# sigma0-dev/polymath

Hardware: AMD Instinct MI355X
Metric: prove_constraints_per_sec (higher is better)
Workload: dtype u32; 1 GPU; 2^20-100-constraint synthetic R1CS (random A*B=C gates), bls12_381, n=2^21, transcript=merlin; msm_pairs_per_proof=29359963, parallelism=one GPU

## Files before the change

polymath_amd/csrc/api.hip:

```cpp
#include <algorithm>
#include <atomic>
#include <cstdlib>
#include <cstring>
#include <exception>
#include <memory>
#include <new>
#include <thread>

#include "internal.h"
#include "comm.h"
#include "fq28.cuh"
#include "../host/hashes.hpp"

using namespace pm;

extern "C" void pm_host_keccak_f1600(uint64_t state[25]) { pmhost::keccak_f1600(state); }

template <class F>
static void parallel_chunks(uint64_t count, F body) {
    unsigned T = std::thread::hardware_concurrency();
    if (T > 32) T = 32;
    if (T < 1 || count < ((uint64_t)1 << 16)) T = 1;
    static const int env_threads = [] { const char *e = getenv("PM_HOST_THREADS"); return e ? std::max(1, atoi(e)) : 0; }();
    if (env_threads) T = (unsigned)env_threads;
// ... 43 lines not shown
struct OptionSpec { const char *env; long long def, lo, hi; };
static const OptionSpec OPTION_SPECS[PM_NUM_OPTIONS] = {
     {"PM_MSM_OVERLAP", 1, 0, 1},
     {"PM_NTT_OVERLAP", 1, 0, 1},
     {"PM_TABLES", PM_TABLES_AUTO, PM_TABLES_OFF, PM_TABLES_NO_WIDE},
     {"PM_MSM_MAX_PIECE_LOG", 27, 4, 27},
     {"PM_MAX_SEG_LOG", 0, 0, 40},
     {"PM_INFLIGHT_CONTEXTS", 1, 1, 64},
     {"PM_MSM_SEG", 0, 0, 1 << 20},
     {"PM_TABLE_C", 0, 0, 24},
     {"PM_WIRE_CHUNK_LOG", 20, 4, 24},
};
static void options_defaults(pm_options *o) {
    for (int k = 0; k < PM_NUM_OPTIONS; ++k) {
        long long v = OPTION_SPECS[k].def;
        if (const char *e = getenv(OPTION_SPECS[k].env)) {
            if (k == PM_OPT_TABLES) v = e[0] == 'w' ? PM_TABLES_WIDE : e[0] == '0' ? PM_TABLES_OFF : PM_TABLES_AUTO;
            else v = atoll(e);
            if (v < OPTION_SPECS[k].lo || v > OPTION_SPECS[k].hi) v = OPTION_SPECS[k].def;
        }
        o->v[k] = v;
    }
    if (o->v[PM_OPT_TABLES] == PM_TABLES_AUTO) {
        const char *e = getenv("PM_WIDE");
        if (e && e[0] == '0') o->v[PM_OPT_TABLES] = PM_TABLES_NO_WIDE;
    }
}

extern "C" int pm_ctx_set_option(pm_ctx *ctx, int option, long long value) {
    if (!ctx || option < 0 || option >= PM_NUM_OPTIONS) return PM_ERR_INVALID_ARG;
    if (value < OPTION_SPECS[option].lo || value > OPTION_SPECS[option].hi) return PM_ERR_INVALID_ARG;
    ctx->opt.v[option] = value;
    if (ctx->aux) ctx->aux->opt.v[option] = value;
    return PM_OK;
}
extern "C" int pm_ctx_get_option(const pm_ctx *ctx, int option, long long *value) {
    if (!ctx || !value || option < 0 || option >= PM_NUM_OPTIONS) return PM_ERR_INVALID_ARG;
    *value = ctx->opt.v[option];
    return PM_OK;
}

extern "C" int pm_ctx_create(int device, pm_ctx **out) {
    if (!out) return PM_ERR_INVALID_ARG;
    *out = nullptr;
    int n = 0;
    if (hipGetDeviceCount(&n) != hipSuccess || n <= 0) return PM_ERR_NO_DEVICE;
    if (device < 0 || device >= n) return PM_ERR_INVALID_ARG;
    pm_ctx *ctx = new (std::nothrow) pm_ctx();
    if (!ctx) return PM_ERR_INVALID_ARG;
    ctx->device = device;
    options_defaults(&ctx->opt);
    ctx->pk = nullptr;
    ctx->phase = 0;
    ctx->aux = nullptr;
    ctx->comm = nullptr;
    ctx->tw_clock = 0;
    ctx->shard_roots_n = 0; ctx->shard_roots_N = 0; ctx->shard_roots_curve = -1;
    ctx->ntt_lds_attr[0] = ctx->ntt_lds_attr[1] = false;
    ctx->h_pinned = nullptr;
    ctx->msm_async = 0;
    ctx->keep_timings = false;
    ctx->lazy_timings = false;
    timing_reset(ctx);
    if (hipSetDevice(device) != hipSuccess || hipStreamCreateWithFlags(&ctx->stream, hipStreamNonBlocking) != hipSuccess) {
        delete ctx;
        return PM_ERR_HIP;
    }
    if (hipEventCreateWithFlags(&ctx->ev_sc_a, hipEventDisableTiming) != hipSuccess) {
        (void)hipStreamDestroy(ctx->stream);
        delete ctx;
        return PM_ERR_HIP;
    }
    *out = ctx;
    return PM_OK;
}

extern "C" void pm_ctx_destroy(pm_ctx *ctx) {
    if (!ctx) return;
    if (ctx->aux) pm_ctx_destroy(ctx->aux);
    (void)hipSetDevice(ctx->device);
    (void)hipStreamSynchronize(ctx->stream);
    timing_flush(ctx);
    MsmWorkspace &m = ctx->msm;
    for (DevBuf *b : {&m.set.sorted, &m.set.counts, &m.set.bucket_off, &m.set.task_off, &m.set.order, &m.set.partials, &m.set.task_cnt}) b->release();
    for (DevBuf *b : {&m.digits, &m.cursor, &m.wsum,
                      &m.region, &m.sub, &m.digits2, &m.len_bins, &m.block_cnt, &m.hot, &ctx->scratch, &ctx->flags, &ctx->xw, &ctx->ue, &ctx->we, &ctx->u, &ctx->w,
                      &ctx->wit_u, &ctx->u2, &ctx->sc_a, &ctx->sc_c, &ctx->quotient, &ctx->ztail, &ctx->ra, &ctx->sh_a, &ctx->sh_b, &ctx->sh_c, &ctx->halo,
                      &ctx->shard_roots, &ctx->ntt_tmp})
        b->release();
    for (auto &b : ctx->lvl) b.release();
    for (auto &b : ctx->fb_table) b.release();
    for (auto &t : ctx->tw) { t.fwd.release(); t.inv.release(); t.fwd_int.release(); t.inv_int.release(); }
    if (ctx->h_pinned) (void)hipHostFree(ctx->h_pinned);
    for (auto &t : ctx->pending_timers) { (void)hipEventDestroy(t.a); (void)hipEventDestroy(t.b); }
    for (hipEvent_t e : ctx->event_pool) (void)hipEventDestroy(e);
    (void)hipEventDestroy(ctx->ev_sc_a);
    (void)hipStreamDestroy(ctx->stream);
    delete ctx;
}

extern "C" const char *pm_last_error(const pm_ctx *ctx) { return ctx ? ctx->err.c_str() : "null context"; }

extern "C" int pm_last_timings(pm_ctx *ctx, double *ms_out, int n_slots) {
    if (!ctx || !ms_out) return PM_ERR_INVALID_ARG;
    if (!ctx->pending_timers.empty()) {
        if (hipSetDevice(ctx->device) != hipSuccess) return PM_ERR_HIP;
        timing_flush_now(ctx);
    }
    for (int i = 0; i < n_slots; ++i) ms_out[i] = i < T_NUM_SLOTS ? ctx->timing_ms[i] : 0.0;
    return PM_OK;
}

template <class C>
static int ntt_host(pm_ctx *ctx, uint64_t *data, unsigned log_n, int inverse) {
    typedef Fp<typename C::FrP> Fr;
    if (log_n > (unsigned)C::TWO_ADICITY) return PM_ERR_DOMAIN_TOO_LARGE;
    size_t bytes = sizeof(Fr) << log_n;
    PM_HIP(ctx, ctx->scratch.reserve(bytes));
    PM_HIP(ctx, hipMemcpyAsync(ctx->scratch.p, data, bytes, hipMemcpyHostToDevice, ctx->stream));
    timing_reset(ctx);
    PM_TRY(ntt_run<C>(ctx, ctx->scratch.as<Fr>(), log_n, inverse != 0));
    PM_HIP(ctx, hipMemcpyAsync(data, ctx->scratch.p, bytes, hipMemcpyDeviceToHost, ctx->stream));
    PM_HIP(ctx, hipStreamSynchronize(ctx->stream));
    timing_flush(ctx);
    return PM_OK;
}

extern "C" int pm_ntt(pm_ctx *ctx, int curve, uint64_t *data, unsigned log_n, int inverse) {
    if (!ctx || !data) return PM_ERR_INVALID_ARG;
    PM_TRY(set_device(ctx));
    return PM_DISPATCH(curve, ntt_host<BlsCurve>(ctx, data, log_n, inverse), ntt_host<BnCurve>(ctx, data, log_n, inverse));
}

template <class C>
static int ntt_dev(pm_ctx *ctx, uint64_t *d, unsigned log_n, int inverse) {
    timing_reset(ctx);
    PM_TRY(ntt_run<C>(ctx, (Fp<typename C::FrP> *)d, log_n, inverse != 0));
    PM_HIP(ctx, hipStreamSynchronize(ctx->stream));
    timing_flush(ctx);
    return PM_OK;
}

extern "C" int pm_ntt_device(pm_ctx *ctx, int curve, uint64_t *d_data, unsigned log_n, int inverse) {
    if (!ctx || !d_data) return PM_ERR_INVALID_ARG;
    PM_TRY(set_device(ctx));
    return PM_DISPATCH(curve, ntt_dev<BlsCurve>(ctx, d_data, log_n, inverse), ntt_dev<BnCurve>(ctx, d_data, log_n, inverse));
}

struct BasesDeleter {
    void operator()(pm_bases *b) const {
        if (!b) return;
        (void)hipSetDevice(b->device);
        if (b->d_points) (void)hipFree(b->d_points);
        if (b->d_inf) (void)hipFree(b->d_inf);
        if (b->d_table) (void)hipFree(b->d_table);
        delete b;
    }
};
typedef std::unique_ptr<pm_bases, BasesDeleter> BasesPtr;

template <class C>
static int bases_upload_impl(pm_ctx *ctx, const void *bases, size_t stride, size_t len, pm_bases **out) {
    if (stride < sizeof(Affine<C>)) return PM_ERR_INVALID_ARG;
    BasesPtr b(new pm_bases{C::ID, ctx->device, len, nullptr});
    if (len) {
        std::vector<Affine<C>> packed(len);
        repack_bases<C>(bases, stride, len, packed.data());
// ... 914 lines not shown
```

polymath_amd/csrc/internal.h:

```cpp
#pragma once
#include <hip/hip_runtime.h>
#include <stdint.h>
#include <stdlib.h>

#include <chrono>
#include <condition_variable>
#include <cstdio>
#include <functional>
#include <mutex>
#include <string>
#include <thread>
#include <vector>

#include "../../include/polymath_hip.h"
#include "../host/layout.hpp"
#include "ec.cuh"

namespace pm {

struct pm_error_sink {
    std::string msg;
};

#define PM_HIP(ctx, expr)                                                                        \
    do {                                                                                         \
        hipError_t _e = (expr);                                                                  \
        if (_e != hipSuccess) {                                                                  \
            (ctx)->err = std::string(#expr) + ": " + hipGetErrorString(_e) + " @" + __FILE__ + ":" + \
                         std::to_string(__LINE__);                                               \
            return PM_ERR_HIP;                                                                   \
        }                                                                                        \
    } while (0)

#define PM_TRY(expr)                  \
    do {                              \
        int _s = (expr);              \
        if (_s != PM_OK) return _s;   \
    } while (0)

struct DevBuf {
    void *p = nullptr;
    size_t bytes = 0;
    hipError_t reserve(size_t need) {
        if (need <= bytes) return hipSuccess;
        if (p) {
            hipError_t e = hipFree(p);
            if (e != hipSuccess) return e;
            p = nullptr;
            bytes = 0;
        }
        size_t want = need + need / 8;
        hipError_t e = hipMalloc(&p, want);
        if (e != hipSuccess) {
            e = hipMalloc(&p, need);
            want = need;
        }
        if (e == hipSuccess) bytes = want;
        return e;
    }
    void release() {
        if (p) (void)hipFree(p);
        p = nullptr;
        bytes = 0;
    }
    template <class T>
    T *as() const { return (T *)p; }
};

enum TimingSlot {
    T_WITNESS_MAP = 0,
    T_NTT = 1,
    T_POLY = 2,
    T_MSM_SORT = 3,
    T_MSM_ACCUMULATE = 4,
    T_MSM_REDUCE = 5,
    T_MSM_TOTAL = 6,
    T_PHASE = 7,
    T_NUM_SLOTS = 8
};

struct MsmSet {
    DevBuf sorted, counts, bucket_off, task_off, order, partials, task_cnt;
};
struct MsmWorkspace {
    MsmSet set;
    DevBuf digits, cursor, wsum, region, sub, digits2, len_bins, block_cnt, hot;
};

struct MsmTables {
    unsigned c = 0, nwin = 0;
    unsigned off[33] = {0};
    unsigned char width[32] = {0};
    size_t stride = 0;
    size_t base_index = 0;
    const unsigned char *inf = nullptr;
    const void *table = nullptr;
    bool wide = false;
};

struct TwiddleCache {
    int curve = -1;
    unsigned log_n = 0;
    unsigned long long stamp = 0;
    DevBuf fwd, inv;
    DevBuf fwd_int, inv_int;
};

}

struct pm_bases {
    int curve;
    int device;
    size_t len;
    void *d_points;
    void *d_inf;
    void *d_table;
    pm::MsmTables tables;
};

struct pm_pk {
    int curve, device;
    uint64_t n, m0, mw, nr, sigma;
    unsigned log_n;
    uint64_t omega[4];
    int shard_rank, shard_count;
    uint64_t *d_rowptr[3];
    uint32_t *d_col[3];
    uint64_t *d_val[3];
    uint64_t nnz[3];
    void *d_bases;
    uint64_t base_len[PM_NUM_BASE_VECS];
    uint64_t seg_off[PM_NUM_BASE_VECS];
    uint64_t total_points;
    uint64_t res_lo[3], res_hi[3], res_dev_off[3];
    uint64_t msm_lo[3], msm_len[3];
    int layout;
    std::vector<pmlayout::Piece> pieces[3];
    uint64_t res_cnt[3];
    std::vector<pmlayout::Segment> segs;
    uint64_t max_seg;
    uint64_t max_piece = (uint64_t)1 << 27;
    struct SegRef { uint64_t a, b; uint32_t rank, idx; };
    std::vector<SegRef> all_segs;
    size_t seg_slots;
    void *d_segs;
    void *d_all_segs = nullptr;
    pm::MsmTables tables[3];
    void *d_tab[3], *d_tab_inf[3];
};

struct pm_worker {
    std::thread th;
    std::mutex mu;
    std::condition_variable cv;
    std::function<void()> job;
    bool has_job = false, done = true, stop = false;
    bool submit(std::function<void()> fn) {
        std::unique_lock<std::mutex> lk(mu);
        if (!th.joinable()) {
            try {
                th = std::thread([this] {
                    std::unique_lock<std::mutex> l(mu);
                    for (;;) {
                        cv.wait(l, [this] { return has_job || stop; });
                        if (stop) return;
// ... 284 lines not shown
```

polymath_amd/csrc/msm.hip:

```cpp
#include <cstdlib>
#include <cstring>

#include "internal.h"
#include "fq28.cuh"

namespace pm {

constexpr uint32_t DIGIT_NONE = 0xFFFFFFFFu;

struct MsmPlan {
    unsigned c, nwin, nbuckets;
    unsigned seg;
    size_t len;
    unsigned chunk, nchunks;
    size_t max_tasks;
};

static MsmPlan make_plan(size_t len, unsigned scalar_bits, unsigned task_len = 0) {
    MsmPlan p;
    p.len = len;
    double best = 1e300;
    unsigned bc = 4;
    for (unsigned c = 4; c <= 16; ++c) {
        unsigned w = (scalar_bits + 1 + c - 1) / c;
// ... 104 lines not shown
        __syncthreads();
        s_a[tid] += va;
        s_b[tid] += vb;
        __syncthreads();
    }
    uint32_t ra = s_a[tid] - sa, rb = s_b[tid] - sb;
#pragma unroll
    for (unsigned k = 0; k < SCAN_PER; ++k) {
        if (base + k < G) { bucket_off[base + k] = ra; task_off[base + k] = rb; }
        ra += c[k];
        rb += nt[k];
    }
    if (tid == 255) { tile_tot[2 * blockIdx.x] = s_a[255]; tile_tot[2 * blockIdx.x + 1] = s_b[255]; }
}

__global__ __launch_bounds__(1024) void k_scan_totals(uint32_t *tile_tot, unsigned ntiles, uint32_t *bucket_off,
                                                      uint32_t *task_off, size_t G) {
    __shared__ uint32_t s_a[1024], s_b[1024];
    const unsigned tid = threadIdx.x;
    uint32_t carry_a = 0, carry_b = 0;
    for (unsigned base = 0; base < ntiles; base += 1024) {
        unsigned i = base + tid;
        uint32_t a = i < ntiles ? tile_tot[2 * i] : 0u, b = i < ntiles ? tile_tot[2 * i + 1] : 0u;
        s_a[tid] = a;
        s_b[tid] = b;
        __syncthreads();
        for (unsigned off = 1; off < 1024; off <<= 1) {
            uint32_t va = 0, vb = 0;
            if (tid >= off) { va = s_a[tid - off]; vb = s_b[tid - off]; }
            __syncthreads();
            s_a[tid] += va;
            s_b[tid] += vb;
            __syncthreads();
        }
        if (i < ntiles) { tile_tot[2 * i] = carry_a + s_a[tid] - a; tile_tot[2 * i + 1] = carry_b + s_b[tid] - b; }
        carry_a += s_a[1023];
        carry_b += s_b[1023];
        __syncthreads();
    }
    if (tid == 0) { bucket_off[G] = carry_a; task_off[G] = carry_b; }
}

__global__ __launch_bounds__(256) void k_scan_add(uint32_t *bucket_off, uint32_t *task_off, const uint32_t *tile_tot, size_t G) {
    const size_t base = (size_t)blockIdx.x * SCAN_TILE + (size_t)threadIdx.x * SCAN_PER;
    const uint32_t oa = tile_tot[2 * blockIdx.x], ob = tile_tot[2 * blockIdx.x + 1];
#pragma unroll
    for (unsigned k = 0; k < SCAN_PER; ++k)
        if (base + k < G) { bucket_off[base + k] += oa; task_off[base + k] += ob; }
}

__global__ __launch_bounds__(1024) void k_scatter(const uint32_t *digits, const uint32_t *bucket_off, uint32_t *cursor,
                                                  uint32_t *sorted, size_t len, unsigned chunk, unsigned nbuckets) {
    extern __shared__ __attribute__((aligned(16))) unsigned char smem_raw[];
    uint32_t *h = (uint32_t *)smem_raw;
    const unsigned w = blockIdx.y;
    for (unsigned b = threadIdx.x; b < nbuckets; b += blockDim.x) h[b] = 0;
    __syncthreads();
    size_t lo = (size_t)blockIdx.x * chunk, hi = lo + chunk;
    if (hi > len) hi = len;
    const uint32_t *d = digits + (size_t)w * len;
    for (size_t i = lo + threadIdx.x; i < hi; i += blockDim.x) {
        uint32_t v = d[i];
        if (v != DIGIT_NONE) atomicAdd(&h[v >> 1], 1u);
    }
    __syncthreads();
    const size_t gbase = (size_t)w * nbuckets;
    for (unsigned b = threadIdx.x; b < nbuckets; b += blockDim.x) {
        uint32_t v = h[b];
        if (v) h[b] = bucket_off[gbase + b] + atomicAdd(&cursor[gbase + b], v);
    }
    __syncthreads();
    for (size_t i = lo + threadIdx.x; i < hi; i += blockDim.x) {
        uint32_t v = d[i];
        if (v != DIGIT_NONE) {
            uint32_t pos = atomicAdd(&h[v >> 1], 1u);
            sorted[pos] = ((uint32_t)i << 1) | (v & 1u);
        }
    }
}

constexpr unsigned TASK_MAX_BINS = 8192;

template <bool SCATTER>
__global__ __launch_bounds__(1024) void k_task_bins(const uint32_t *counts, const uint32_t *task_off, size_t G, unsigned seg,
                                                    unsigned lshift, unsigned nbins, uint32_t *len_cnt, const uint32_t *len_off,
                                                    uint32_t *len_cursor, uint32_t *order) {
    extern __shared__ __attribute__((aligned(16))) unsigned char smem_raw[];
    uint32_t *h = (uint32_t *)smem_raw;
    for (unsigned b = threadIdx.x; b < nbins; b += blockDim.x) h[b] = 0;
    __syncthreads();
    const size_t g = (size_t)blockIdx.x * blockDim.x + threadIdx.x;
    uint32_t t0 = 0, n = 0, rank_full = 0, rank_last = 0;
    unsigned bin = 0;
    if (g < G) {
        t0 = task_off[g];
        n = task_off[g + 1] - t0;
        if (n) {
            const uint32_t L = counts[g] - (n - 1) * seg;
            bin = (seg - L) >> lshift;
            if (n > 1) rank_full = atomicAdd(&h[0], n - 1);
            rank_last = atomicAdd(&h[bin], 1u);
        }
    }
    __syncthreads();
    if (!SCATTER) {
        for (unsigned b = threadIdx.x; b < nbins; b += blockDim.x) {
            const uint32_t v = h[b];
            if (v) atomicAdd(&len_cnt[b], v);
        }
    } else {
        for (unsigned b = threadIdx.x; b < nbins; b += blockDim.x) {
            const uint32_t v = h[b];
            if (v) h[b] = len_off[b] + atomicAdd(&len_cursor[b], v);
        }
        __syncthreads();
        if (n) {
            const uint32_t at = h[0] + rank_full;
            for (uint32_t k = 0; k + 1 < n; ++k) order[at + k] = t0 + k;
            order[h[bin] + rank_last] = t0 + n - 1;
        }
    }
}

template <class C, bool TABLE>
__global__ __launch_bounds__(128) void k_accumulate(const uint32_t *sorted, const uint32_t *counts,
                                                    const uint32_t *bucket_off, const uint32_t *task_off,
                                                    const uint32_t *order, const void *points, XYZZ<C> *partials, size_t G,
                                                    unsigned seg) {
    typedef typename C::FqRR RR;
    size_t t = (size_t)blockIdx.x * blockDim.x + threadIdx.x;
    const uint32_t total = task_off[G];
    if (t >= total) return;
    t = order[t];
    size_t lo = 0, hi = G;
    while (hi - lo > 1) {
        size_t mid = (lo + hi) >> 1;
        if (task_off[mid] <= t) lo = mid; else hi = mid;
    }
    const size_t g = lo;
    const uint32_t k = (uint32_t)t - task_off[g];
    const uint32_t start = bucket_off[g] + k * seg;
    uint32_t end = bucket_off[g] + counts[g];
    if (start + seg < end) end = start + seg;
    XYZZ28<C> acc;
    acc.X = acc.Y = acc.ZZ = acc.ZZZ = f28_zero<RR>();
#ifndef PM_ACC_IDX_VEC
#define PM_ACC_IDX_VEC 4
#endif
#if PM_ACC_IDX_VEC == 4
    uint4 quad = make_uint4(0u, 0u, 0u, 0u);
    uint32_t quad_at = 0xffffffffu;
#endif
    for (uint32_t e = start; e < end; ++e) {
#if PM_ACC_IDX_VEC == 4
        if ((e & ~3u) != quad_at) {
            quad_at = e & ~3u;
            quad = *(const uint4 *)(sorted + quad_at);
        }
        const unsigned q = e & 3u;
        const uint32_t v = q == 0 ? quad.x : q == 1 ? quad.y : q == 2 ? quad.z : quad.w;
#else
        const uint32_t v = sorted[e];
#endif
        const bool neg = (v & 1u) != 0;
        if (TABLE) {
            const TablePoint<C> tp = ((const TablePoint<C> *)points)[v >> 1];
            F28<RR> x2, y2;
#pragma unroll
            for (int i = 0; i < RR::N; ++i) { x2.l[i] = tp.x[i]; y2.l[i] = tp.y[i]; }
            if (!xyzz28_madd_limbs<C>(acc, x2, y2, neg)) acc = xyzz28_madd_exceptional<C>(acc, table_point_to_affine<C>(tp), neg);
        } else {
            const Affine<C> p = ((const Affine<C> *)points)[v >> 1];
            if (!xyzz28_madd<C>(acc, p, neg)) acc = xyzz28_madd_exceptional<C>(acc, p, neg);
        }
    }
    partials[t] = xyzz28_store<C>(acc);
}

constexpr unsigned RED_K = 4;

template <class C>
__device__ __forceinline__ void lds_tree_sum(XYZZ28<C> *sh) {
    __syncthreads();
    for (unsigned off = blockDim.x >> 1; off > 0; off >>= 1) {
        if (threadIdx.x < off) {
            const XYZZ28<C> b = sh[threadIdx.x + off];
            xyzz28_add_into_full<C>(&sh[threadIdx.x], b);
        }
        __syncthreads();
    }
}

constexpr uint32_t FOLD_MIN = 8, FOLD_BLOCK_MIN = 1024;

__global__ void k_task_counts(const uint32_t *task_off, size_t G, uint32_t *task_cnt, uint32_t *hot_a, uint32_t *hot_b,
                              uint32_t *hot_counts , uint32_t cap) {
    size_t g = (size_t)blockIdx.x * blockDim.x + threadIdx.x;
    if (g >= G) return;
    const uint32_t n = task_off[g + 1] - task_off[g];
    task_cnt[g] = n;
    if (n > FOLD_BLOCK_MIN) {
        const uint32_t i = atomicAdd(&hot_counts[0], 1u);
        if (i < cap) hot_a[i] = (uint32_t)g;
    } else if (n > FOLD_MIN) {
        const uint32_t i = atomicAdd(&hot_counts[1], 1u);
        if (i < cap) hot_b[i] = (uint32_t)g;
    }
}

template <class C, unsigned LANES>
__global__ __launch_bounds__(256) __attribute__((amdgpu_waves_per_eu(2, 2))) void k_task_fold(XYZZ<C> *partials, const uint32_t *task_off, uint32_t *task_cnt,
                                                   const uint32_t *hot, const uint32_t *hot_count, uint32_t cap) {
    extern __shared__ __attribute__((aligned(16))) unsigned char smem_raw[];
    XYZZ28<C> *sh = (XYZZ28<C> *)smem_raw;
    typedef typename C::FqRR RR;
    uint32_t listed = *hot_count;
    if (listed > cap) listed = cap;
    constexpr unsigned GROUPS = 256 / LANES;
    const unsigned group = threadIdx.x / LANES, lane = threadIdx.x % LANES;
    for (uint32_t h0 = blockIdx.x * GROUPS; h0 < listed; h0 += gridDim.x * GROUPS) {
        const uint32_t h = h0 + group;
        XYZZ28<C> *acc = &sh[threadIdx.x];
        acc->X = acc->Y = acc->ZZ = acc->ZZZ = f28_zero<RR>();
        uint32_t first = 0, n = 0;
        if (h < listed) {
            first = task_off[hot[h]];
            n = task_off[hot[h] + 1] - first;
            for (uint32_t i = lane; i < n; i += LANES) xyzz28_add_into_full<C>(acc, xyzz28_load<C>(partials[first + i]));
        }
        __syncthreads();
        for (unsigned off = LANES >> 1; off > 0; off >>= 1) {
            if (lane < off) {
                const XYZZ28<C> b = sh[threadIdx.x + off];
                xyzz28_add_into_full<C>(&sh[threadIdx.x], b);
            }
            __syncthreads();
        }
        if (h < listed && lane == 0) {
            partials[first] = xyzz28_store<C>(sh[threadIdx.x]);
            task_cnt[hot[h]] = 1;
        }
        __syncthreads();
    }
}

template <class C>
__global__ __launch_bounds__(256) __attribute__((amdgpu_waves_per_eu(2, 2))) void k_bucket_reduce(const XYZZ<C> *partials, const uint32_t *task_off, const uint32_t *task_cnt, unsigned nbuckets,
                                                       unsigned lanes_per_window, unsigned bpw, XYZZ<C> *out) {
    extern __shared__ __attribute__((aligned(16))) unsigned char smem_raw[];
    XYZZ28<C> *sh = (XYZZ28<C> *)smem_raw;
    typedef typename C::FqRR RR;
    const unsigned w = blockIdx.x / bpw, bw = blockIdx.x % bpw;
    const unsigned j = bw * blockDim.x + threadIdx.x;
    XYZZ28<C> run;
    run.X = run.Y = run.ZZ = run.ZZZ = f28_zero<RR>();
    XYZZ28<C> *acc = &sh[threadIdx.x];
    *acc = run;
    if (j < lanes_per_window) {
        const size_t gbase = (size_t)w * nbuckets + (size_t)j * RED_K;
// ... 456 lines not shown
            if ((vm >> q) & 1u) {
                const uint32_t slot = h[key[q] >> bin_shift] + rank[q];
                st_key[slot] = key[q];
                st_val[slot] = val[q];
            }
        }
        __syncthreads();
        for (uint32_t i = t; i < cnt; i += ST_THREADS) {
            const uint16_t k = st_key[i];
            const uint32_t pos = delta[k >> bin_shift] + i;
            if (MODE == RS_FINAL) {
                sorted[pos] = st_val[i];
            } else {
                keys_out[pos] = k & low_mask;
                vals_out[pos] = st_val[i];
            }
        }
        __syncthreads();
    }
}

__global__ __launch_bounds__(1024) void k_scan_small(const uint32_t *cnt, uint32_t *off, uint32_t *zero, unsigned n) {
    __shared__ uint32_t s[1024];
    __shared__ uint32_t carry;
    const unsigned t = threadIdx.x;
    if (t == 0) carry = 0;
    __syncthreads();
    for (unsigned base = 0; base < n; base += 1024) {
        const unsigned i = base + t;
        const uint32_t v = i < n ? cnt[i] : 0u;
        s[t] = v;
        __syncthreads();
        for (unsigned o = 1; o < 1024; o <<= 1) {
            uint32_t a = t >= o ? s[t - o] : 0u;
            __syncthreads();
            s[t] += a;
            __syncthreads();
        }
        if (i < n) { off[i] = carry + s[t] - v; zero[i] = 0; }
        __syncthreads();
        if (t == 1023) carry += s[1023];
        __syncthreads();
    }
    if (t == 0) off[n] = carry;
}

template <class C>
static void host_finish(const XYZZ<C> *S , unsigned nwin, unsigned c, Affine<C> *out, int *inf) {
    XYZZ<C> acc = XYZZ<C>::identity();
    for (int w = (int)nwin - 1; w >= 0; --w) {
        for (unsigned k = 0; k < c; ++k) acc = xyzz_dbl<C>(acc);
        acc = xyzz_add<C>(acc, xyzz_internal_to_std<C>(S[w]));
    }
    *inf = acc.is_identity() ? 1 : 0;
    *out = xyzz_to_affine<C>(acc);
}

template <class C>
static int fold_hot_buckets(pm_ctx *ctx, MsmSet &S, size_t G, size_t max_tasks) {
    MsmWorkspace &ws = ctx->msm;
    size_t cap = max_tasks > G ? max_tasks - G + 1 : 1;
    cap = cap / FOLD_MIN + 1;
    PM_HIP(ctx, S.task_cnt.reserve(G * 4));
    PM_HIP(ctx, ws.hot.reserve((2 * cap + 2) * 4));
    uint32_t *hot_counts = ws.hot.as<uint32_t>(), *hot_a = hot_counts + 2, *hot_b = hot_a + cap;
    PM_HIP(ctx, hipMemsetAsync(hot_counts, 0, 8, ctx->stream));
    hipLaunchKernelGGL(k_task_counts, dim3((unsigned)((G + 255) / 256)), dim3(256), 0, ctx->stream, S.task_off.as<uint32_t>(), G,
                       S.task_cnt.as<uint32_t>(), hot_a, hot_b, hot_counts, (uint32_t)cap);
    PM_HIP(ctx, hipGetLastError());
    hipLaunchKernelGGL((k_task_fold<C, 256>), dim3(256), dim3(256), 256 * sizeof(XYZZ28<C>), ctx->stream, S.partials.as<XYZZ<C>>(),
                       S.task_off.as<uint32_t>(), S.task_cnt.as<uint32_t>(), hot_a, hot_counts, (uint32_t)cap);
    PM_HIP(ctx, hipGetLastError());
    hipLaunchKernelGGL((k_task_fold<C, 64>), dim3(1024), dim3(256), 256 * sizeof(XYZZ28<C>), ctx->stream, S.partials.as<XYZZ<C>>(),
                       S.task_off.as<uint32_t>(), S.task_cnt.as<uint32_t>(), hot_b, hot_counts + 1, (uint32_t)cap);
    PM_HIP(ctx, hipGetLastError());
    return PM_OK;
}

static int task_order(pm_ctx *ctx, MsmSet &S, const uint32_t *counts, size_t G, size_t seg, size_t max_tasks) {
    MsmWorkspace &ws = ctx->msm;
    unsigned lshift = 0;
    while (((seg - 1) >> lshift) + 1 > TASK_MAX_BINS) ++lshift;
    const unsigned nbins = (unsigned)(((seg - 1) >> lshift) + 1);
    PM_HIP(ctx, S.order.reserve(max_tasks * 4));
    PM_HIP(ctx, ws.len_bins.reserve((3 * (size_t)nbins + 4) * 4));
    uint32_t *len_cnt = ws.len_bins.as<uint32_t>(), *len_off = len_cnt + nbins, *len_cursor = len_off + nbins + 1;
    PM_HIP(ctx, hipMemsetAsync(len_cnt, 0, (size_t)nbins * 4, ctx->stream));
    const unsigned blocks = (unsigned)((G + 1023) / 1024);
    hipLaunchKernelGGL(k_task_bins<false>, dim3(blocks), dim3(1024), nbins * 4, ctx->stream, counts, S.task_off.as<uint32_t>(), G,
                       (unsigned)seg, lshift, nbins, len_cnt, (const uint32_t *)nullptr, (uint32_t *)nullptr, (uint32_t *)nullptr);
    PM_HIP(ctx, hipGetLastError());
    hipLaunchKernelGGL(k_scan_small, dim3(1), dim3(1024), 0, ctx->stream, len_cnt, len_off, len_cursor, nbins);
    PM_HIP(ctx, hipGetLastError());
    hipLaunchKernelGGL(k_task_bins<true>, dim3(blocks), dim3(1024), nbins * 4, ctx->stream, counts, S.task_off.as<uint32_t>(), G,
                       (unsigned)seg, lshift, nbins, (uint32_t *)nullptr, len_off, len_cursor, S.order.as<uint32_t>());
    PM_HIP(ctx, hipGetLastError());
    return PM_OK;
}


template <class C>
static int msm_piece(pm_ctx *ctx, const Affine<C> *d_bases, const Fp<typename C::FrP> *d_scalars, size_t len, Affine<C> *h_out,
                     int *h_inf) {
    typedef typename C::FrP FrP;
    StageTimer t_total(ctx, T_MSM_TOTAL);
    MsmPlan p = make_plan(len, (unsigned)FrP::BITS, (unsigned)ctx->opt.v[PM_OPT_MSM_TASK_LEN]);
    MsmWorkspace &ws = ctx->msm;
    MsmSet &S = ws.set;
    const size_t G = (size_t)p.nwin * p.nbuckets;
    PM_HIP(ctx, ws.digits.reserve((size_t)p.nwin * len * 4));
    PM_HIP(ctx, S.sorted.reserve((size_t)p.nwin * len * 4 + 16));
    PM_HIP(ctx, S.counts.reserve(2 * G * 4));
    PM_HIP(ctx, S.bucket_off.reserve((G + 1) * 4));
    PM_HIP(ctx, S.task_off.reserve((G + 1) * 4));
    PM_HIP(ctx, ws.cursor.reserve(((G + SCAN_TILE - 1) / SCAN_TILE + 1) * 8));
    PM_HIP(ctx, S.partials.reserve(p.max_tasks * sizeof(XYZZ<C>)));
    const unsigned red_lanes = (p.nbuckets + RED_K - 1) / RED_K;
    unsigned red_block = 64;
    while (red_block < red_lanes && red_block < 256) red_block <<= 1;
    const unsigned bpw = (red_lanes + red_block - 1) / red_block;
    PM_HIP(ctx, ws.wsum.reserve(((size_t)p.nwin * bpw + p.nwin) * sizeof(XYZZ<C>)));
    uint32_t *counts = S.counts.as<uint32_t>(), *cursor = counts + G;
    {
        StageTimer t(ctx, T_MSM_SORT);
        PM_HIP(ctx, hipMemsetAsync(counts, 0, 2 * G * 4, ctx->stream));
        hipLaunchKernelGGL(k_digits<C>, dim3((unsigned)((len + 255) / 256)), dim3(256), 0, ctx->stream, d_scalars, d_bases,
                           ws.digits.as<uint32_t>(), len, p.c, p.nwin);
        PM_HIP(ctx, hipGetLastError());
        size_t lds = (size_t)p.nbuckets * 4;
        if (lds > 48 * 1024) {
            PM_HIP(ctx, hipFuncSetAttribute((const void *)k_hist, hipFuncAttributeMaxDynamicSharedMemorySize, (int)lds));
            PM_HIP(ctx, hipFuncSetAttribute((const void *)k_scatter, hipFuncAttributeMaxDynamicSharedMemorySize, (int)lds));
        }
        hipLaunchKernelGGL(k_hist, dim3(p.nchunks, p.nwin), dim3(1024), lds, ctx->stream, ws.digits.as<uint32_t>(), counts,
                           len, p.chunk, p.nbuckets);
        PM_HIP(ctx, hipGetLastError());
        const unsigned ntiles = (unsigned)((G + SCAN_TILE - 1) / SCAN_TILE);
        hipLaunchKernelGGL(k_scan_tiles, dim3(ntiles), dim3(256), 0, ctx->stream, counts, S.bucket_off.as<uint32_t>(),
                           S.task_off.as<uint32_t>(), ws.cursor.as<uint32_t>(), G, p.seg);
        PM_HIP(ctx, hipGetLastError());
        hipLaunchKernelGGL(k_scan_totals, dim3(1), dim3(1024), 0, ctx->stream, ws.cursor.as<uint32_t>(), ntiles,
                           S.bucket_off.as<uint32_t>(), S.task_off.as<uint32_t>(), G);
        PM_HIP(ctx, hipGetLastError());
        hipLaunchKernelGGL(k_scan_add, dim3(ntiles), dim3(256), 0, ctx->stream, S.bucket_off.as<uint32_t>(),
                           S.task_off.as<uint32_t>(), ws.cursor.as<uint32_t>(), G);
        PM_HIP(ctx, hipGetLastError());
        hipLaunchKernelGGL(k_scatter, dim3(p.nchunks, p.nwin), dim3(1024), lds, ctx->stream, ws.digits.as<uint32_t>(),
                           S.bucket_off.as<uint32_t>(), cursor, S.sorted.as<uint32_t>(), len, p.chunk, p.nbuckets);
        PM_HIP(ctx, hipGetLastError());
        PM_TRY(task_order(ctx, S, counts, G, p.seg, p.max_tasks));
    }
    {
        StageTimer t(ctx, T_MSM_ACCUMULATE);
        size_t blocks = (p.max_tasks + 127) / 128;
        hipLaunchKernelGGL((k_accumulate<C, false>), dim3((unsigned)blocks), dim3(128), 0, ctx->stream, S.sorted.as<uint32_t>(),
                           counts, S.bucket_off.as<uint32_t>(), S.task_off.as<uint32_t>(), S.order.as<uint32_t>(), (const void *)d_bases,
                           S.partials.as<XYZZ<C>>(), G, p.seg);
        PM_HIP(ctx, hipGetLastError());
    }
    std::vector<XYZZ<C>> hS(p.nwin);
    {
        StageTimer t(ctx, T_MSM_REDUCE);
        PM_TRY(fold_hot_buckets<C>(ctx, S, G, p.max_tasks));
        XYZZ<C> *parts = ws.wsum.as<XYZZ<C>>(), *dS = parts + (size_t)p.nwin * bpw;
        hipLaunchKernelGGL(k_bucket_reduce<C>, dim3(p.nwin * bpw), dim3(red_block), red_block * sizeof(XYZZ28<C>), ctx->stream,
                           S.partials.as<XYZZ<C>>(), S.task_off.as<uint32_t>(), S.task_cnt.as<uint32_t>(), p.nbuckets, red_lanes, bpw, parts);
        PM_HIP(ctx, hipGetLastError());
        hipLaunchKernelGGL(k_sum_parts<C>, dim3(p.nwin), dim3(64), 0, ctx->stream, parts, bpw, dS);
        PM_HIP(ctx, hipGetLastError());
        PM_HIP(ctx, hipMemcpyAsync(hS.data(), dS, hS.size() * sizeof(XYZZ<C>), hipMemcpyDeviceToHost, ctx->stream));
    }
    PM_HIP(ctx, hipStreamSynchronize(ctx->stream));
    host_finish<C>(hS.data(), p.nwin, p.c, h_out, h_inf);
    return PM_OK;
}

template <class C>
static int msm_piece_tables(pm_ctx *ctx, const MsmTables &tb, const Fp<typename C::FrP> *d_scalars,
                            size_t len, Affine<C> *h_out, int *h_inf, const Affine<C> *plain = nullptr, XYZZ<C> *async_res = nullptr) {
    typedef typename C::FrP FrP;
    StageTimer t_total(ctx, T_MSM_TOTAL);
    MsmWorkspace &ws = ctx->msm;
    const unsigned c = tb.c, nwin = tb.nwin;
    const bool wide = tb.wide;
    if ((wide && !plain) || (wide && async_res)) return PM_ERR_INVALID_ARG;
    const size_t NB1 = (size_t)1 << (c - 1);
    const size_t NBn = wide ? wide_narrow_buckets(nwin, c) : 0;
    const unsigned n_wide_sets = !wide ? 1u : (NBn == NB1 ? nwin : 256 % nwin), n_narrow_sets = wide ? nwin - n_wide_sets : 0u;
    const size_t NB = (size_t)n_wide_sets * NB1 + (size_t)n_narrow_sets * NBn;
    const uint32_t win_buckets = wide ? (uint32_t)NB1 : 0u, narrow_buckets = (uint32_t)NBn;
    const unsigned lo_buckets = (unsigned)(NB < ((size_t)1 << LO_BITS) ? NB : ((size_t)1 << LO_BITS));
    const unsigned regions = (unsigned)(NB / lo_buckets);
    if (regions > 1024 || (size_t)regions * lo_buckets != NB) return PM_ERR_INVALID_ARG;
    for (unsigned w = 0; w < nwin; ++w)
        if (tb.off[w] != win_off(nwin, w) || tb.width[w] != win_width(nwin, w)) return PM_ERR_INVALID_ARG;
    const bool two_level = NB1 >= 4096;
    if (wide && !two_level) return PM_ERR_INVALID_ARG;
    const size_t Emax = (size_t)nwin * len;
    size_t seg = 2 * (Emax / NB + 1);
    if (seg < 64) seg = 64;
    if (ctx->opt.v[PM_OPT_MSM_TASK_LEN] > 0) seg = (size_t)ctx->opt.v[PM_OPT_MSM_TASK_LEN];
    const size_t max_tasks = NB + Emax / seg + 1;
    const unsigned chunk = 1u << RS_CHUNK_LOG;
    const size_t keys_bytes = (Emax * 2 + 15) & ~(size_t)15;
    PM_HIP(ctx, ws.digits.reserve(keys_bytes + Emax * 4 + 128));
    PM_HIP(ctx, ws.region.reserve((3 * (size_t)regions + 4) * 4));
    PM_HIP(ctx, ws.cursor.reserve(((NB + SCAN_TILE - 1) / SCAN_TILE + 1) * 8));
    MsmSet &S = ws.set;
    {
        PM_HIP(ctx, S.sorted.reserve(Emax * 4 + 16));
        PM_HIP(ctx, S.counts.reserve(2 * NB * 4));
        PM_HIP(ctx, S.bucket_off.reserve((NB + 1) * 4));
        PM_HIP(ctx, S.task_off.reserve((NB + 1) * 4));
        PM_HIP(ctx, S.partials.reserve(max_tasks * sizeof(XYZZ<C>)));
        PM_HIP(ctx, S.task_cnt.reserve(NB * 4));
    }
    const unsigned red_lanes = (unsigned)((NB + RED_K - 1) / RED_K);
    unsigned red_block = 64;
    while (red_block < red_lanes && red_block < 256) red_block <<= 1;
    const unsigned bpw = (red_lanes + red_block - 1) / red_block;
    if (!two_level) PM_HIP(ctx, ws.wsum.reserve(((size_t)bpw + 4) * sizeof(XYZZ<C>)));
    uint16_t *keys = (uint16_t *)ws.digits.p;
    uint32_t *vals = (uint32_t *)((uint8_t *)ws.digits.p + keys_bytes);
    uint32_t *region_count = ws.region.as<uint32_t>(), *region_off = region_count + regions, *region_cursor = region_off + regions + 1;
#ifndef PM_PARTITION_LANES
#define PM_PARTITION_LANES 512
#endif
#ifndef PM_PARTITION_WIDE_LANES
#define PM_PARTITION_WIDE_LANES 1024
#endif
#ifndef PM_PARTITION_WIDE_FROM
#define PM_PARTITION_WIDE_FROM 512
#endif
    const unsigned pbd = regions >= PM_PARTITION_WIDE_FROM ? PM_PARTITION_WIDE_LANES : nwin <= 16 ? PM_PARTITION_LANES : 256;
    if (regions > 2 * pbd) return PM_ERR_INVALID_ARG;
    const size_t plds = 2 * 1024 * 4 + (size_t)pbd * nwin * 8;
    {
        const unsigned pblocks_max = (unsigned)((len + pbd - 1) / pbd);
        const BlockScanShape bsh_max = block_scan_shape(pblocks_max, regions);
        PM_HIP(ctx, ws.block_cnt.reserve(((size_t)pblocks_max + bsh_max.G) * regions * 4));
    }
// ... 17 lines not shown
        const unsigned pblocks = (unsigned)((cnt + pbd - 1) / pbd);
        const BlockScanShape bsh = block_scan_shape(pblocks, regions);
        uint32_t *block_cnt = ws.block_cnt.as<uint32_t>(), *block_partial = block_cnt + (size_t)pblocks * regions;
        int launched = 0;
#define PM_TBL_CASE(NW)                                                                                                     \
        case NW:                                                                                                                \
            hipLaunchKernelGGL((k_tbl_count<FrP, NW>), dim3(pblocks), dim3(pbd), 0, st, sc, inf, cnt, regions,                  \
                               block_cnt, win_buckets, narrow_buckets);                                                         \
            hipLaunchKernelGGL(k_block_sums, dim3(bsh.G), dim3(1024), 0, st, block_cnt, pblocks, regions, bsh, block_partial);  \
            hipLaunchKernelGGL(k_block_offsets, dim3(bsh.G), dim3(1024), 0, st, block_cnt, pblocks, regions, bsh, block_partial, \
                               region_count);                                                                                  \
            hipLaunchKernelGGL(k_region_offsets, dim3(1), dim3(1024), 0, st, region_count, region_off, region_cursor,           \
                               regions);                                                                                        \
            if (hipFuncSetAttribute((const void *)k_tbl_partition<FrP, NW>, hipFuncAttributeMaxDynamicSharedMemorySize,         \
                                    (int)plds) != hipSuccess) break;                                                            \
            hipLaunchKernelGGL((k_tbl_partition<FrP, NW>), dim3(pblocks), dim3(pbd), plds, st, sc, inf, cnt,                    \
                               regions, region_off, block_cnt, wide ? (size_t)0 : tb.stride, tb.base_index + lo, keys, vals,    \
                               win_buckets, narrow_buckets);                                                                    \
            launched = 1;                                                                                                       \
            break;
        switch (nwin) {
            PM_TBL_CASE(10) PM_TBL_CASE(11) PM_TBL_CASE(12) PM_TBL_CASE(13) PM_TBL_CASE(14) PM_TBL_CASE(15) PM_TBL_CASE(16)
            PM_TBL_CASE(17) PM_TBL_CASE(18) PM_TBL_CASE(19) PM_TBL_CASE(20) PM_TBL_CASE(21) PM_TBL_CASE(22) PM_TBL_CASE(23)
            PM_TBL_CASE(24) PM_TBL_CASE(25) PM_TBL_CASE(26) PM_TBL_CASE(27) PM_TBL_CASE(28) PM_TBL_CASE(29) PM_TBL_CASE(30)
            PM_TBL_CASE(31) PM_TBL_CASE(32)
            default: break;
        }
#undef PM_TBL_CASE
        if (!launched) return PM_ERR_INVALID_ARG;
        PM_HIP(ctx, hipGetLastError());
        const unsigned sblocks = (unsigned)((E + chunk - 1) / chunk);
        const unsigned ntiles = (unsigned)((NB + SCAN_TILE - 1) / SCAN_TILE);
        auto bucket_scan = [&]() -> int {
            hipLaunchKernelGGL(k_scan_tiles, dim3(ntiles), dim3(256), 0, st, counts, S.bucket_off.as<uint32_t>(),
                               S.task_off.as<uint32_t>(), ws.cursor.as<uint32_t>(), NB, (unsigned)seg);
            PM_HIP(ctx, hipGetLastError());
            hipLaunchKernelGGL(k_scan_totals, dim3(1), dim3(1024), 0, st, ws.cursor.as<uint32_t>(), ntiles,
                               S.bucket_off.as<uint32_t>(), S.task_off.as<uint32_t>(), NB);
            PM_HIP(ctx, hipGetLastError());
            hipLaunchKernelGGL(k_scan_add, dim3(ntiles), dim3(256), 0, st, S.bucket_off.as<uint32_t>(),
                               S.task_off.as<uint32_t>(), ws.cursor.as<uint32_t>(), NB);
            PM_HIP(ctx, hipGetLastError());
            return PM_OK;
        };
        if (lo_buckets == (1u << LO_BITS)) {
            uint32_t *sub_count = ws.sub.as<uint32_t>(), *sub_off = sub_count + nsub, *sub_cursor = sub_off + nsub + 1;
            uint16_t *keys2 = (uint16_t *)ws.digits2.p;
            uint32_t *vals2 = (uint32_t *)((uint8_t *)ws.digits2.p + keys_bytes);
            PM_HIP(ctx, hipMemsetAsync(sub_count, 0, (size_t)nsub * 4, st));
            hipLaunchKernelGGL(k_hist_small, dim3(sblocks), dim3(1024), 0, st, keys, region_off, regions, FIN_BITS, SUB_BINS, chunk,
                               sub_count);
            PM_HIP(ctx, hipGetLastError());
            hipLaunchKernelGGL(k_scan_small, dim3(1), dim3(1024), 0, st, sub_count, sub_off, sub_cursor, nsub);
            PM_HIP(ctx, hipGetLastError());
            const unsigned stblocks = (unsigned)((E + ST_CHUNK - 1) / ST_CHUNK);
            hipLaunchKernelGGL(k_region_pass_staged<RS_MID>, dim3(stblocks), dim3(ST_THREADS), 0, st, keys, vals, region_off, regions,
                               FIN_BITS, SUB_BINS, sub_off, sub_cursor, (uint32_t *)nullptr, keys2, vals2);
            PM_HIP(ctx, hipGetLastError());
            hipLaunchKernelGGL(k_hist_small, dim3(sblocks), dim3(1024), 0, st, keys2, sub_off, nsub, 0u, FIN_BINS, chunk, counts);
            PM_HIP(ctx, hipGetLastError());
            PM_TRY(bucket_scan());
            hipLaunchKernelGGL(k_region_pass_staged<RS_FINAL>, dim3(stblocks), dim3(ST_THREADS), 0, st, keys2, vals2, sub_off, nsub, 0u,
                               FIN_BINS, S.bucket_off.as<uint32_t>(), cursor, S.sorted.as<uint32_t>(), (uint16_t *)nullptr,
                               (uint32_t *)nullptr);
            PM_HIP(ctx, hipGetLastError());
        } else {
            const size_t lds = (size_t)lo_buckets * 4;
            hipLaunchKernelGGL(k_region_pass<RS_HIST>, dim3(sblocks), dim3(1024), lds, st, keys, vals, region_off, regions, 0u,
                               lo_buckets, chunk, counts, (const uint32_t *)nullptr, (uint32_t *)nullptr, (uint32_t *)nullptr,
                               (uint16_t *)nullptr, (uint32_t *)nullptr);
            PM_HIP(ctx, hipGetLastError());
            PM_TRY(bucket_scan());
            hipLaunchKernelGGL(k_region_pass<RS_FINAL>, dim3(sblocks), dim3(1024), lds, st, keys, vals, region_off, regions, 0u,
                               lo_buckets, chunk, (uint32_t *)nullptr, S.bucket_off.as<uint32_t>(), cursor, S.sorted.as<uint32_t>(),
                               (uint16_t *)nullptr, (uint32_t *)nullptr);
            PM_HIP(ctx, hipGetLastError());
        }
        PM_TRY(task_order(ctx, S, counts, NB, seg, max_tasks));
        return PM_OK;
    };
    PM_TRY(sort_all());
    {
        StageTimer t(ctx, T_MSM_ACCUMULATE);
        const size_t blocks = (max_tasks + 127) / 128;
        if (wide)
            hipLaunchKernelGGL((k_accumulate<C, false>), dim3((unsigned)blocks), dim3(128), 0, ctx->stream, S.sorted.as<uint32_t>(), S.counts.as<uint32_t>(),
                               S.bucket_off.as<uint32_t>(), S.task_off.as<uint32_t>(), S.order.as<uint32_t>(), (const void *)plain,
                               S.partials.as<XYZZ<C>>(), NB, (unsigned)seg);
        else
            hipLaunchKernelGGL((k_accumulate<C, true>), dim3((unsigned)blocks), dim3(128), 0, ctx->stream, S.sorted.as<uint32_t>(), S.counts.as<uint32_t>(),
                               S.bucket_off.as<uint32_t>(), S.task_off.as<uint32_t>(), S.order.as<uint32_t>(), tb.table,
                               S.partials.as<XYZZ<C>>(), NB, (unsigned)seg);
        PM_HIP(ctx, hipGetLastError());
    }
    if (wide) {
        std::vector<XYZZ<C>> hS(nwin);
        {
            StageTimer t(ctx, T_MSM_REDUCE);
            PM_TRY(fold_hot_buckets<C>(ctx, S, NB, max_tasks));
            XYZZ<C> *dres = nullptr;
            PM_TRY(reduce_two_level<C>(ctx, NB1, &dres, n_wide_sets));
            PM_HIP(ctx, hipMemcpyAsync(hS.data(), dres, n_wide_sets * sizeof(XYZZ<C>), hipMemcpyDeviceToHost, ctx->stream));
            if (n_narrow_sets) {
                PM_TRY(reduce_two_level<C>(ctx, NBn, &dres, n_narrow_sets, (size_t)n_wide_sets * NB1));
                PM_HIP(ctx, hipMemcpyAsync(hS.data() + n_wide_sets, dres, n_narrow_sets * sizeof(XYZZ<C>), hipMemcpyDeviceToHost, ctx->stream));
            }
        }
        PM_HIP(ctx, hipStreamSynchronize(ctx->stream));
        XYZZ<C> acc = XYZZ<C>::identity();
        for (int w = (int)nwin - 1; w >= 0; --w) {
            for (unsigned b = 0; b < tb.width[w]; ++b) acc = xyzz_dbl<C>(acc);
            acc = xyzz_add<C>(acc, xyzz_internal_to_std<C>(hS[w]));
        }
        *h_inf = acc.is_identity() ? 1 : 0;
        *h_out = xyzz_to_affine<C>(acc);
        return PM_OK;
    }
    XYZZ<C> hres;
    {
        StageTimer t(ctx, T_MSM_REDUCE);
        PM_TRY(fold_hot_buckets<C>(ctx, S, NB, max_tasks));
        XYZZ<C> *dres = nullptr;
        if (two_level) {
            PM_TRY(reduce_two_level<C>(ctx, NB, &dres));
        } else {
            XYZZ<C> *parts = ws.wsum.as<XYZZ<C>>();
            dres = parts + bpw;
            hipLaunchKernelGGL(k_bucket_reduce<C>, dim3(bpw), dim3(red_block), red_block * sizeof(XYZZ28<C>), ctx->stream,
                               S.partials.as<XYZZ<C>>(), S.task_off.as<uint32_t>(), S.task_cnt.as<uint32_t>(), (unsigned)NB, red_lanes, bpw, parts);
            PM_HIP(ctx, hipGetLastError());
            hipLaunchKernelGGL(k_sum_parts<C>, dim3(1), dim3(64), 0, ctx->stream, parts, bpw, dres);
            PM_HIP(ctx, hipGetLastError());
        }
        PM_HIP(ctx, hipMemcpyAsync(async_res ? async_res : &hres, dres, sizeof(hres), hipMemcpyDeviceToHost, ctx->stream));
    }
    if (async_res) return PM_OK;
    PM_HIP(ctx, hipStreamSynchronize(ctx->stream));
    XYZZ<C> acc = xyzz_internal_to_std<C>(hres);
    *h_inf = acc.is_identity() ? 1 : 0;
    *h_out = xyzz_to_affine<C>(acc);
    return PM_OK;
}

template <class C>
int msm_run(pm_ctx *ctx, const Affine<C> *d_bases, const Fp<typename C::FrP> *d_scalars, size_t len, Affine<C> *h_out,
            int *h_inf, const MsmTables *tables) {
    if (len == 0) {
        *h_out = Affine<C>::infinity();
        *h_inf = 1;
        return PM_OK;
    }
    const bool tbl = tables && tables->c;
    const size_t MSM_MAX_PIECE = msm_max_piece(ctx);
    const bool wide = tbl && tables->wide;
    if (len <= MSM_MAX_PIECE)
        return tbl ? msm_piece_tables<C>(ctx, *tables, d_scalars, len, h_out, h_inf, wide ? d_bases : nullptr)
                   : msm_piece<C>(ctx, d_bases, d_scalars, len, h_out, h_inf);
    XYZZ<C> acc = XYZZ<C>::identity();
    for (size_t off = 0; off < len; off += MSM_MAX_PIECE) {
        size_t cnt = len - off < MSM_MAX_PIECE ? len - off : MSM_MAX_PIECE;
        Affine<C> part;
        int inf = 1;
        if (tbl) {
            MsmTables tb = *tables;
            tb.base_index += off;
            PM_TRY(msm_piece_tables<C>(ctx, tb, d_scalars + off, cnt, &part, &inf, wide ? d_bases : nullptr));
        } else {
            PM_TRY(msm_piece<C>(ctx, d_bases + off, d_scalars + off, cnt, &part, &inf));
        }
        if (!inf) xyzz_madd<C>(acc, part, false);
    }
    *h_inf = acc.is_identity() ? 1 : 0;
    *h_out = xyzz_to_affine<C>(acc);
    return PM_OK;
}

// ... 43 lines not shown
```

Before: 17.35 million constraints/s.

## Precompute MSM task descriptors and use persistent atomic-ticket accumulate kernel

The task binning pass now writes a uint4 descriptor per task (partial index, start, end) instead of a bare task id. This removes the per-thread binary search over task_off and the extra counts/bucket_off loads in the accumulate kernel. Accumulation becomes a persistent kernel sized to occupancy, where each wavefront grabs 64 tasks at a time from a global atomic ticket to balance uneven task lengths. The cost is four times more task-buffer memory traffic and a global atomic per wavefront batch, plus host-side occupancy queries on every launch.

```diff
diff --git a/polymath_amd/csrc/api.hip b/polymath_amd/csrc/api.hip
--- a/polymath_amd/csrc/api.hip
+++ b/polymath_amd/csrc/api.hip
@@ -149,7 +149,7 @@
     (void)hipStreamSynchronize(ctx->stream);
     timing_flush(ctx);
     MsmWorkspace &m = ctx->msm;
-    for (DevBuf *b : {&m.set.sorted, &m.set.counts, &m.set.bucket_off, &m.set.task_off, &m.set.order, &m.set.partials, &m.set.task_cnt}) b->release();
+    for (DevBuf *b : {&m.set.sorted, &m.set.counts, &m.set.bucket_off, &m.set.task_off, &m.set.tasks, &m.set.partials, &m.set.task_cnt}) b->release();
     for (DevBuf *b : {&m.digits, &m.cursor, &m.wsum,
                       &m.region, &m.sub, &m.digits2, &m.len_bins, &m.block_cnt, &m.hot, &ctx->scratch, &ctx->flags, &ctx->xw, &ctx->ue, &ctx->we, &ctx->u, &ctx->w,
                       &ctx->wit_u, &ctx->u2, &ctx->sc_a, &ctx->sc_c, &ctx->quotient, &ctx->ztail, &ctx->ra, &ctx->sh_a, &ctx->sh_b, &ctx->sh_c, &ctx->halo,
diff --git a/polymath_amd/csrc/internal.h b/polymath_amd/csrc/internal.h
--- a/polymath_amd/csrc/internal.h
+++ b/polymath_amd/csrc/internal.h
@@ -80,7 +80,7 @@
 };
 
 struct MsmSet {
-    DevBuf sorted, counts, bucket_off, task_off, order, partials, task_cnt;
+    DevBuf sorted, counts, bucket_off, task_off, tasks, partials, task_cnt;
 };
 struct MsmWorkspace {
     MsmSet set;
diff --git a/polymath_amd/csrc/msm.hip b/polymath_amd/csrc/msm.hip
--- a/polymath_amd/csrc/msm.hip
+++ b/polymath_amd/csrc/msm.hip
@@ -210,21 +210,22 @@
 constexpr unsigned TASK_MAX_BINS = 8192;
 
 template <bool SCATTER>
-__global__ __launch_bounds__(1024) void k_task_bins(const uint32_t *counts, const uint32_t *task_off, size_t G, unsigned seg,
-                                                    unsigned lshift, unsigned nbins, uint32_t *len_cnt, const uint32_t *len_off,
-                                                    uint32_t *len_cursor, uint32_t *order) {
+__global__ __launch_bounds__(1024) void k_task_bins(const uint32_t *counts, const uint32_t *bucket_off, const uint32_t *task_off, size_t G,
+                                                    unsigned seg, unsigned lshift, unsigned nbins, uint32_t *len_cnt, const uint32_t *len_off,
+                                                    uint32_t *len_cursor, uint4 *tasks) {
     extern __shared__ __attribute__((aligned(16))) unsigned char smem_raw[];
     uint32_t *h = (uint32_t *)smem_raw;
     for (unsigned b = threadIdx.x; b < nbins; b += blockDim.x) h[b] = 0;
     __syncthreads();
     const size_t g = (size_t)blockIdx.x * blockDim.x + threadIdx.x;
-    uint32_t t0 = 0, n = 0, rank_full = 0, rank_last = 0;
+    uint32_t t0 = 0, n = 0, rank_full = 0, rank_last = 0, cnt = 0;
     unsigned bin = 0;
     if (g < G) {
         t0 = task_off[g];
         n = task_off[g + 1] - t0;
         if (n) {
-            const uint32_t L = counts[g] - (n - 1) * seg;
+            cnt = counts[g];
+            const uint32_t L = cnt - (n - 1) * seg;
             bin = (seg - L) >> lshift;
             if (n > 1) rank_full = atomicAdd(&h[0], n - 1);
             rank_last = atomicAdd(&h[bin], 1u);
@@ -243,33 +244,17 @@
         }
         __syncthreads();
         if (n) {
-            const uint32_t at = h[0] + rank_full;
-            for (uint32_t k = 0; k + 1 < n; ++k) order[at + k] = t0 + k;
-            order[h[bin] + rank_last] = t0 + n - 1;
+            const uint32_t at = h[0] + rank_full, first = bucket_off[g];
+            for (uint32_t k = 0; k + 1 < n; ++k)
+                tasks[at + k] = make_uint4(t0 + k, first + k * seg, first + (k + 1) * seg, 0u);
+            tasks[h[bin] + rank_last] = make_uint4(t0 + n - 1, first + (n - 1) * seg, first + cnt, 0u);
         }
     }
 }
 
 template <class C, bool TABLE>
-__global__ __launch_bounds__(128) void k_accumulate(const uint32_t *sorted, const uint32_t *counts,
-                                                    const uint32_t *bucket_off, const uint32_t *task_off,
-                                                    const uint32_t *order, const void *points, XYZZ<C> *partials, size_t G,
-                                                    unsigned seg) {
+__device__ __forceinline__ void accumulate_task(const uint32_t *sorted, const uint4 d, const void *points, XYZZ<C> *partials) {
     typedef typename C::FqRR RR;
-    size_t t = (size_t)blockIdx.x * blockDim.x + threadIdx.x;
-    const uint32_t total = task_off[G];
-    if (t >= total) return;
-    t = order[t];
-    size_t lo = 0, hi = G;
-    while (hi - lo > 1) {
-        size_t mid = (lo + hi) >> 1;
-        if (task_off[mid] <= t) lo = mid; else hi = mid;
-    }
-    const size_t g = lo;
-    const uint32_t k = (uint32_t)t - task_off[g];
-    const uint32_t start = bucket_off[g] + k * seg;
-    uint32_t end = bucket_off[g] + counts[g];
-    if (start + seg < end) end = start + seg;
     XYZZ28<C> acc;
     acc.X = acc.Y = acc.ZZ = acc.ZZZ = f28_zero<RR>();
 #ifndef PM_ACC_IDX_VEC
@@ -279,7 +264,7 @@
     uint4 quad = make_uint4(0u, 0u, 0u, 0u);
     uint32_t quad_at = 0xffffffffu;
 #endif
-    for (uint32_t e = start; e < end; ++e) {
+    for (uint32_t e = d.y; e < d.z; ++e) {
 #if PM_ACC_IDX_VEC == 4
         if ((e & ~3u) != quad_at) {
             quad_at = e & ~3u;
@@ -302,7 +287,22 @@
             if (!xyzz28_madd<C>(acc, p, neg)) acc = xyzz28_madd_exceptional<C>(acc, p, neg);
         }
     }
-    partials[t] = xyzz28_store<C>(acc);
+    partials[d.x] = xyzz28_store<C>(acc);
+}
+
+template <class C, bool TABLE>
+__global__ __launch_bounds__(128) void k_accumulate(const uint32_t *sorted, const uint32_t *task_off, const uint4 *tasks,
+                                                    const void *points, XYZZ<C> *partials, size_t G, uint32_t *ticket) {
+    const uint32_t total = task_off[G];
+    const unsigned lane = threadIdx.x & 63u;
+    for (;;) {
+        uint32_t base = 0;
+        if (lane == 0) base = atomicAdd(ticket, 64u);
+        base = __builtin_amdgcn_readfirstlane(base);
+        if (base >= total) break;
+        const uint32_t i = base + lane;
+        if (i < total) accumulate_task<C, TABLE>(sorted, tasks[i], points, partials);
+    }
 }
 
 constexpr unsigned RED_K = 4;
@@ -925,18 +925,33 @@
     unsigned lshift = 0;
     while (((seg - 1) >> lshift) + 1 > TASK_MAX_BINS) ++lshift;
     const unsigned nbins = (unsigned)(((seg - 1) >> lshift) + 1);
-    PM_HIP(ctx, S.order.reserve(max_tasks * 4));
-    PM_HIP(ctx, ws.len_bins.reserve((3 * (size_t)nbins + 4) * 4));
-    uint32_t *len_cnt = ws.len_bins.as<uint32_t>(), *len_off = len_cnt + nbins, *len_cursor = len_off + nbins + 1;
-    PM_HIP(ctx, hipMemsetAsync(len_cnt, 0, (size_t)nbins * 4, ctx->stream));
+    PM_HIP(ctx, S.tasks.reserve(max_tasks * sizeof(uint4)));
+    PM_HIP(ctx, ws.len_bins.reserve((3 * (size_t)nbins + 5) * 4));
+    uint32_t *ticket = ws.len_bins.as<uint32_t>(), *len_cnt = ticket + 1, *len_off = len_cnt + nbins, *len_cursor = len_off + nbins + 1;
+    PM_HIP(ctx, hipMemsetAsync(ticket, 0, ((size_t)nbins + 1) * 4, ctx->stream));
     const unsigned blocks = (unsigned)((G + 1023) / 1024);
-    hipLaunchKernelGGL(k_task_bins<false>, dim3(blocks), dim3(1024), nbins * 4, ctx->stream, counts, S.task_off.as<uint32_t>(), G,
-                       (unsigned)seg, lshift, nbins, len_cnt, (const uint32_t *)nullptr, (uint32_t *)nullptr, (uint32_t *)nullptr);
+    hipLaunchKernelGGL(k_task_bins<false>, dim3(blocks), dim3(1024), nbins * 4, ctx->stream, counts, S.bucket_off.as<uint32_t>(),
+                       S.task_off.as<uint32_t>(), G, (unsigned)seg, lshift, nbins, len_cnt, (const uint32_t *)nullptr, (uint32_t *)nullptr,
+                       (uint4 *)nullptr);
     PM_HIP(ctx, hipGetLastError());
     hipLaunchKernelGGL(k_scan_small, dim3(1), dim3(1024), 0, ctx->stream, len_cnt, len_off, len_cursor, nbins);
     PM_HIP(ctx, hipGetLastError());
-    hipLaunchKernelGGL(k_task_bins<true>, dim3(blocks), dim3(1024), nbins * 4, ctx->stream, counts, S.task_off.as<uint32_t>(), G,
-                       (unsigned)seg, lshift, nbins, (uint32_t *)nullptr, len_off, len_cursor, S.order.as<uint32_t>());
+    hipLaunchKernelGGL(k_task_bins<true>, dim3(blocks), dim3(1024), nbins * 4, ctx->stream, counts, S.bucket_off.as<uint32_t>(),
+                       S.task_off.as<uint32_t>(), G, (unsigned)seg, lshift, nbins, (uint32_t *)nullptr, len_off, len_cursor,
+                       S.tasks.as<uint4>());
+    PM_HIP(ctx, hipGetLastError());
+    return PM_OK;
+}
+
+template <class C, bool TABLE>
+static int accumulate(pm_ctx *ctx, MsmSet &S, const void *points, size_t G, size_t max_tasks) {
+    int per_cu = 0, cus = 0;
+    PM_HIP(ctx, hipOccupancyMaxActiveBlocksPerMultiprocessor(&per_cu, (const void *)k_accumulate<C, TABLE>, 128, 0));
+    PM_HIP(ctx, hipDeviceGetAttribute(&cus, hipDeviceAttributeMultiprocessorCount, ctx->device));
+    size_t blocks = (size_t)(per_cu > 0 ? per_cu : 1) * (size_t)(cus > 0 ? cus : 1);
+    if (blocks > (max_tasks + 127) / 128) blocks = (max_tasks + 127) / 128;
+    hipLaunchKernelGGL((k_accumulate<C, TABLE>), dim3((unsigned)blocks), dim3(128), 0, ctx->stream, S.sorted.as<uint32_t>(),
+                       S.task_off.as<uint32_t>(), S.tasks.as<uint4>(), points, S.partials.as<XYZZ<C>>(), G, ctx->msm.len_bins.as<uint32_t>());
     PM_HIP(ctx, hipGetLastError());
     return PM_OK;
 }
@@ -995,11 +1010,7 @@
     }
     {
         StageTimer t(ctx, T_MSM_ACCUMULATE);
-        size_t blocks = (p.max_tasks + 127) / 128;
-        hipLaunchKernelGGL((k_accumulate<C, false>), dim3((unsigned)blocks), dim3(128), 0, ctx->stream, S.sorted.as<uint32_t>(),
-                           counts, S.bucket_off.as<uint32_t>(), S.task_off.as<uint32_t>(), S.order.as<uint32_t>(), (const void *)d_bases,
-                           S.partials.as<XYZZ<C>>(), G, p.seg);
-        PM_HIP(ctx, hipGetLastError());
+        PM_TRY((accumulate<C, false>(ctx, S, (const void *)d_bases, G, p.max_tasks)));
     }
     std::vector<XYZZ<C>> hS(p.nwin);
     {
@@ -1183,16 +1194,8 @@
     PM_TRY(sort_all());
     {
         StageTimer t(ctx, T_MSM_ACCUMULATE);
-        const size_t blocks = (max_tasks + 127) / 128;
-        if (wide)
-            hipLaunchKernelGGL((k_accumulate<C, false>), dim3((unsigned)blocks), dim3(128), 0, ctx->stream, S.sorted.as<uint32_t>(), S.counts.as<uint32_t>(),
-                               S.bucket_off.as<uint32_t>(), S.task_off.as<uint32_t>(), S.order.as<uint32_t>(), (const void *)plain,
-                               S.partials.as<XYZZ<C>>(), NB, (unsigned)seg);
-        else
-            hipLaunchKernelGGL((k_accumulate<C, true>), dim3((unsigned)blocks), dim3(128), 0, ctx->stream, S.sorted.as<uint32_t>(), S.counts.as<uint32_t>(),
-                               S.bucket_off.as<uint32_t>(), S.task_off.as<uint32_t>(), S.order.as<uint32_t>(), tb.table,
-                               S.partials.as<XYZZ<C>>(), NB, (unsigned)seg);
-        PM_HIP(ctx, hipGetLastError());
+        if (wide) PM_TRY((accumulate<C, false>(ctx, S, (const void *)plain, NB, max_tasks)));
+        else PM_TRY((accumulate<C, true>(ctx, S, tb.table, NB, max_tasks)));
     }
     if (wide) {
         std::vector<XYZZ<C>> hS(nwin);
```

Result: faster. 17.94 million constraints/s, median of 6 (+3.4%).
